# ZINZINBIN/Optimal-Control-1D-Electrostatic-Plasma

Hardware: AMD Instinct MI355X
Metric: particle-steps/sec (N×envs×steps) at N=1e6, Ng=256; % HBM roofline (higher is better)
Workload: dtype f64

## Files before the change

optimal-control-1d-electrostatic-plasma_amd/csrc/pic_device.h:

```cpp
#pragma once
#include <hip/hip_runtime.h>

#include <cmath>
#include <cstdint>
#include <type_traits>

#include "picstep.h"
#include "pic_limits.h"

namespace {

#ifndef PIC_STAMP
#define PIC_STAMP(slot) ((void)0)
#define PIC_STAMP_LOADS(slot) ((void)0)
#endif

constexpr int kInlineDoubles = 32;
struct InlineDoubles { double v[kInlineDoubles]; };

template <typename T>
__device__ __forceinline__ T kernarg_at(size_t offset) {
#if defined(__HIP_DEVICE_COMPILE__)
  using KP = const __attribute__((address_space(4))) char*;
  KP ka = (KP)__builtin_amdgcn_kernarg_segment_ptr();
  asm volatile("" : "+s"(ka));
  T out;
  __builtin_memcpy(&out, (const __attribute__((address_space(4))) T*)(ka + offset), sizeof(T));
  return out;
#else
  (void)offset;
  return T{};
#endif
}

template <typename T>
__device__ __forceinline__ const T* kernarg_ptr(size_t offset) {
#if defined(__HIP_DEVICE_COMPILE__)
  using KP = const __attribute__((address_space(4))) char*;
  KP ka = (KP)__builtin_amdgcn_kernarg_segment_ptr();
  return (const T*)(const char*)(ka + offset);
#else
  (void)offset;
  return nullptr;
#endif
}

template <int BYTES>
__device__ __forceinline__ void kernarg_warm() {
#if defined(__HIP_DEVICE_COMPILE__)
  using KP = const __attribute__((address_space(4))) unsigned*;
  KP ka = (KP)__builtin_amdgcn_kernarg_segment_ptr();
  unsigned w = 0;
#pragma unroll
  for (int line = 1; line < (BYTES + 63) / 64; ++line) w |= ka[line * 16];
  asm volatile("" ::"s"(w));
#endif
}

enum Stage : int {
  ST_A = 0,
  ST_B = 1,
  ST_C = 2,
  ST_D = 3,
  ST_REFRESH = 4,
  ST_PROBE = 5,
  ST_B2 = 6,
  ST_D2 = 7,
  ST_SE = 8,
  ST_FE = 9,
  ST_VK = 10,
  ST_VM = 11,
  ST_C_RO = 12,
  ST_D_RC = 13,
  ST_D2_RC = 14
};

using acc_t = long long;

__device__ __forceinline__ acc_t acc_row_sum(const acc_t* __restrict__ row, int j, int S, long long sub) {
  const acc_t* p = row + j;
  acc_t t = 0;
  int s = 0;
  for (; s + 4 <= S; s += 4) {
    const acc_t r0 = p[0]; p += sub;
    const acc_t r1 = p[0]; p += sub;
    const acc_t r2 = p[0]; p += sub;
    const acc_t r3 = p[0]; p += sub;
    t += (r0 + r1) + (r2 + r3);
  }
  for (; s < S; ++s) { t += p[0]; p += sub; }
  return t;
}

struct SweepArgs {
  long long N;
  long long ld;
  long long chunk;
  int Ng;
  int nblk;
  int R;
  int reverse;
  int fg;
  int S;
  int act_inline;
  long long sub;
  double magic;
  double L, dx, rdx, dt;
  double c_prev, c_cur, d_cur, c_next, d_prev;
  double scale, n0;
  double to_units;
  double N_over_L;
};

struct SolveArgs {
  long long N;
  long long sub;
  int Ng;
  int nblk;
  int fg;
  int S;
  double L, dx, n0;
  double scale;
  double N_over_L;
};

struct AccRequest { acc_t r[4]; };
__device__ __forceinline__ AccRequest acc_row_request(const acc_t* __restrict__ row, int j, int S, long long sub) {
  AccRequest q;
#pragma unroll
  for (int s = 0; s < 4; ++s) q.r[s] = row[(size_t)(s < S ? s : 0) * sub + j];
  return q;
}
__device__ __forceinline__ acc_t acc_row_finish(const AccRequest& q, int S) {
  return (q.r[0] + (S > 1 ? q.r[1] : 0)) + ((S > 2 ? q.r[2] : 0) + (S > 3 ? q.r[3] : 0));
}

struct Control {
  const double* ext;
  const double* act;
  const double* basis;
  int M;
};

__device__ __forceinline__ double actuator_field(const double* __restrict__ bc, const double* __restrict__ bs,
                                                 const double* __restrict__ a, int j, int M) {
  double c = 0.0, s = 0.0;
  for (int m = 0; m < M; ++m) c += bc[(size_t)j * M + m] * a[m];
  for (int m = 0; m < M; ++m) s += bs[(size_t)j * M + m] * a[M + m];
  return c + s;
}

typedef double pic_v2d __attribute__((ext_vector_type(2)));
typedef float pic_v4f __attribute__((ext_vector_type(4)));
typedef unsigned pic_v4u __attribute__((ext_vector_type(4)));

struct PosF64 { using X = double;   using V = double; using W = double; using XV = pic_v2d; using VV = pic_v2d; static constexpr int VEC = 2; static constexpr bool kFixed = false; };
struct PosF32 { using X = float;    using V = float;  using W = float;  using XV = pic_v4f; using VV = pic_v4f; static constexpr int VEC = 4; static constexpr bool kFixed = false; };
struct PosU32 { using X = unsigned; using V = float;  using W = float;  using XV = pic_v4u; using VV = pic_v4f; static constexpr int VEC = 4; static constexpr bool kFixed = true; };

template <typename VT>
__device__ __forceinline__ VT stream_load(const VT* p) { return *p; }

struct StreamOut {
  __amdgpu_buffer_rsrc_t rsrc;
  __device__ explicit StreamOut(void* base) : rsrc(__builtin_amdgcn_make_buffer_rsrc(base, 0, 0x7fffffff, 0x00020000)) {}
  template <typename VT>
  __device__ __forceinline__ void store(int off, VT v) const {
    static_assert(sizeof(VT) == 16, "particle tiles are 16 bytes per lane");
    typedef unsigned pic_v4raw __attribute__((ext_vector_type(4)));
    pic_v4raw w;
    __builtin_memcpy(&w, &v, 16);
    __builtin_amdgcn_raw_buffer_store_b128(w, rsrc, off, 0, 16);
  }
};

template <typename P>
struct Consts {
  typename P::W L, dx, rdx, dt, c_prev, c_cur, d_cur, c_next, d_prev;
  float to_units;
  double magic;
  int Ng;
  __device__ explicit Consts(const SweepArgs& a)
      : L((typename P::W)a.L), dx((typename P::W)a.dx), rdx((typename P::W)a.rdx), dt((typename P::W)a.dt),
        c_prev((typename P::W)a.c_prev), c_cur((typename P::W)a.c_cur), d_cur((typename P::W)a.d_cur),
        c_next((typename P::W)a.c_next), d_prev((typename P::W)a.d_prev), to_units((float)a.to_units), magic(a.magic), Ng(a.Ng) {}
  __device__ Consts(double L_, double dx_, int Ng_)
      : L((typename P::W)L_), dx((typename P::W)dx_), rdx((typename P::W)1 / (typename P::W)dx_), dt(0), c_prev(0),
        c_cur(0), d_cur(0), c_next(0), d_prev(0), to_units((float)(4294967296.0 / L_)), magic(0), Ng(Ng_) {}
};

template <typename T>
__device__ __noinline__ T wrap_periodic_far(T q, T L) {
  T r = fmod(q, L);
  if (r < T(0)) {
    r += L;
    if (r >= L) r = T(0);
  } else if (r == T(0)) {
    r = T(0);
  }
  return r;
}

template <typename T>
__device__ __forceinline__ T wrap_periodic(T q, T L, unsigned& bad) {
  if (__builtin_amdgcn_ballot_w64(!(q > T(0) && q < L)) == 0) return q;
  T up = q + L;
  up = (up >= L) ? T(0) : up;
  T r = (q <= T(0)) ? up : q;
  r = (q >= L) ? q - L : r;
  if (__builtin_expect(!(r >= T(0) && r < L), 0)) {
    r = wrap_periodic_far(q, L);
    if (!(r >= T(0) && r < L)) {
      bad += 1u;
      r = T(0);
    }
  }
  return r;
}

template <typename T>
__device__ __forceinline__ T div_dx(T a, T dx, T rdx) {
  T q0 = a * rdx;
  T rem = fma(-q0, dx, a);
  return fma(rem, rdx, q0);
}

template <typename P, int SHAPE>
__device__ __forceinline__ void locate_in_box(typename P::X xw, const Consts<P>& k, int& j, typename P::W (&w)[3], unsigned& frac) {
  using T = typename P::W;
  static_assert(!P::kFixed, "fixed-point positions need no wrap: locate() is the whole of it");
  frac = 0u;
  T jf = floor(div_dx(xw, k.dx, k.rdx));
  j = (int)jf;
  if ((unsigned)j >= (unsigned)k.Ng) j = 0;
  if (SHAPE == PIC_CIC) {
    w[0] = div_dx((jf + T(1)) * k.dx - xw, k.dx, k.rdx);
    w[1] = div_dx(xw - jf * k.dx, k.dx, k.rdx);
    w[2] = T(0);
  } else {
    T d = div_dx(xw - jf * k.dx, k.dx, k.rdx);
    T a = T(1.5) - d, b = d - T(1), c = d - T(0.5);
    w[0] = T(0.5) * (a * a);
    w[1] = T(0.75) - b * b;
    w[2] = T(0.5) * (c * c);
  }
}

template <typename P, int SHAPE>
__device__ __forceinline__ void locate(typename P::X q, const Consts<P>& k, typename P::X& xw, int& j,
                                       typename P::W (&w)[3], unsigned& frac, unsigned& bad) {
  using T = typename P::W;
  if constexpr (P::kFixed) {
    xw = q;
    j = (int)__umulhi(q, (unsigned)k.Ng);
    frac = q * (unsigned)k.Ng;
    const T d = (T)frac * T(2.3283064365386963e-10);
    if (SHAPE == PIC_CIC) {
      w[1] = d;
      w[0] = T(1) - d;
      w[2] = T(0);
    } else {
      T a = T(1.5) - d, b = d - T(1), c = d - T(0.5);
      w[0] = T(0.5) * (a * a);
      w[1] = T(0.75) - b * b;
      w[2] = T(0.5) * (c * c);
    }
  } else {
    xw = wrap_periodic(q, k.L, bad);
    locate_in_box<P, SHAPE>(xw, k, j, w, frac);
  }
}

template <typename P>
__device__ __forceinline__ double pos_to_length(typename P::X q, double L) {
  if constexpr (P::kFixed) return (double)q * (L * 2.3283064365386963e-10);
  else return (double)q;
}

template <typename P>
__device__ __forceinline__ typename P::X pos_from_length(double xs, double L, unsigned& bad) {
  if constexpr (P::kFixed) {
    double r = xs - floor(xs / L) * L;
    if (!(r >= 0.0 && r < L)) { if (!(r == L)) bad += 1u; r = 0.0; }
    return (unsigned)((unsigned long long)rint(r / L * 4294967296.0) & 0xFFFFFFFFull);
  } else {
    return (typename P::X)xs;
  }
}

template <typename P>
__device__ __forceinline__ typename P::X drift(typename P::X q, typename P::V p, typename P::W c, const Consts<P>& k,
                                               unsigned& bad) {
  using T = typename P::W;
  if constexpr (P::kFixed) {
    const float d = ((c * (T)p) * k.dt) * k.to_units;
    if (!(fabsf(d) < 2147483648.0f)) bad += 1u;
    return q + (unsigned)__float2int_rn(d);
  } else {
    return q + (c * (T)p) * k.dt;
  }
}

template <typename T, int SHAPE>
__device__ __forceinline__ T gather_field(const T* __restrict__ Es, int j, const T (&w)[3]) {
  T e = w[0] * Es[j] + w[1] * Es[j + 1];
  if (SHAPE == PIC_TSC) e = e + w[2] * Es[j + 2];
  return e;
}

struct fix_t { unsigned long long v; };
constexpr int FX_FRAC = 24;
constexpr int FX_LOW = 44;

__device__ __forceinline__ acc_t to_fixed(double w, double magic) {
  return __double_as_longlong(w + magic) - __double_as_longlong(magic);
}

template <typename A, typename P, int SHAPE>
__device__ __forceinline__ void deposit(A* __restrict__ acc, int j, const typename P::W (&w)[3], unsigned frac,
                                        double magic) {
  if constexpr (std::is_same<A, fix_t>::value) {
    static_assert(SHAPE == PIC_CIC, "the packed accumulator is CIC only");
    unsigned long long lo;
    if constexpr (P::kFixed) {
      lo = (frac >> 8) + ((frac >> 7) & 1u);
    } else {
      const float wr = fminf(fmaxf((float)w[1], 0.0f), 1.0f);
      lo = (unsigned long long)(unsigned)(wr * (float)(1u << FX_FRAC) + 0.5f);
    }
    atomicAdd(reinterpret_cast<unsigned long long*>(acc) + j, (1ull << FX_LOW) + lo);
  } else if constexpr (std::is_same<A, acc_t>::value) {
    unsigned long long* a = reinterpret_cast<unsigned long long*>(acc);
    atomicAdd(a + j, (unsigned long long)to_fixed((double)w[0], magic));
    atomicAdd(a + j + 1, (unsigned long long)to_fixed((double)w[1], magic));
    if (SHAPE == PIC_TSC) atomicAdd(a + j + 2, (unsigned long long)to_fixed((double)w[2], magic));
  } else {
    atomicAdd(&acc[j], (A)w[0]);
    atomicAdd(&acc[j + 1], (A)w[1]);
    if (SHAPE == PIC_TSC) atomicAdd(&acc[j + 2], (A)w[2]);
  }
}

template <int CTRL, int ROW_MASK = 0xF>
__device__ __forceinline__ double dpp_add(double v) {
  const int lo = __builtin_amdgcn_update_dpp(0, __double2loint(v), CTRL, ROW_MASK, 0xF, true);
  const int hi = __builtin_amdgcn_update_dpp(0, __double2hiint(v), CTRL, ROW_MASK, 0xF, true);
  return v + __hiloint2double(hi, lo);
}

__device__ __forceinline__ double wave_incl_scan(double v) {
  v = dpp_add<0x111>(v);
  v = dpp_add<0x112>(v);
  v = dpp_add<0x114>(v);
  v = dpp_add<0x118>(v);
  v = dpp_add<0x142, 0xA>(v);
  v = dpp_add<0x143, 0xC>(v);
  return v;
}

__device__ __forceinline__ double wave_sum(double v) {
  v = wave_incl_scan(v);
  const int lo = __builtin_amdgcn_readlane(__double2loint(v), 63);
  const int hi = __builtin_amdgcn_readlane(__double2hiint(v), 63);
  return __hiloint2double(hi, lo);
}

template <int NW>
__device__ __forceinline__ double block_excl_scan(double v, double* ws, double& total) {
  const int lane = threadIdx.x & 63, w = threadIdx.x >> 6;
  double inc = wave_incl_scan(v);
  if (lane == 63) ws[w] = inc;
  __syncthreads();
  double off = 0.0, tot = 0.0;
  for (int i = 0; i < NW; ++i) {
    double s = ws[i];
    if (i < w) off += s;
    tot += s;
  }
  __syncthreads();
  total = tot;
  return off + (inc - v);
}

template <int NW>
__device__ __forceinline__ double block_sum(double v, double* ws) {
  double w = wave_sum(v);
  if ((threadIdx.x & 63) == 0) ws[threadIdx.x >> 6] = w;
  __syncthreads();
  double s = 0.0;
  for (int i = 0; i < NW; ++i) s += ws[i];
  __syncthreads();
  return s;
}

template <int NW>
__device__ __forceinline__ void block_sum2(double a, double b, double* ws, double& sa, double& sb) {
  const double wa = wave_sum(a), wb = wave_sum(b);
  if ((threadIdx.x & 63) == 0) {
    ws[threadIdx.x >> 6] = wa;
    ws[NW + (threadIdx.x >> 6)] = wb;
  }
  __syncthreads();
  sa = 0.0;
  sb = 0.0;
  for (int i = 0; i < NW; ++i) {
    sa += ws[i];
    sb += ws[NW + i];
  }
  __syncthreads();
}

template <int NW>
__device__ __forceinline__ void mesh_mode(const double* __restrict__ E, const double* __restrict__ twc,
                                          const double* __restrict__ tws, int Ng, double* __restrict__ ws, double& re,
                                          double& im) {
  double sr = 0.0, si = 0.0;
  int t0 = threadIdx.x;
  asm volatile("" : "+v"(t0));
  for (int j = t0; j < Ng; j += NW * 64) {
    const double e = E[j];
    sr += e * twc[j];
    si -= e * tws[j];
  }
  double a, b;
  block_sum2<NW>(sr, si, ws, a, b);
  re = a / Ng * 2.0;
  im = b / Ng * 2.0;
}

struct Feedback {
  const double* tw;
  int rows;
  int M;
  double* act_out;
  double* act_hist;
  const double* gain;
  double* modes;
  double* modes_hist;
};

__device__ __forceinline__ double gain_row(const double* __restrict__ g, const double* __restrict__ m, int n) {
  double acc = 0.0;
  bool any = false;
  for (int k = 0; k < n; ++k) {
    const double gk = g[k];
    if (gk != 0.0) {
      const double t = gk * m[k];
      acc = any ? acc + t : t;
      any = true;
    }
  }
  return acc;
}

template <int NW>
__device__ __forceinline__ void feedback_action(const double* __restrict__ E, const Feedback& fb, int env, int Ng,
                                                double* __restrict__ ws, double* __restrict__ a_lds) {
  const size_t r = (size_t)env * 2 * fb.M;
  for (int m = 0; m < fb.M; ++m) {
    double re, im;
    mesh_mode<NW>(E, fb.tw + (size_t)m * Ng, fb.tw + ((size_t)fb.rows + m) * Ng, Ng, ws, re, im);
    if (threadIdx.x == 0) {
      if (fb.gain) {
        double* mv = a_lds ? a_lds : fb.modes + r;
        mv[m] = re; mv[fb.M + m] = im;
        if (fb.modes_hist) { fb.modes_hist[r + m] = re; fb.modes_hist[r + fb.M + m] = im; }
        continue;
      }
      const double c = -re, s = im;
      if (a_lds) { a_lds[m] = c; a_lds[fb.M + m] = s; }
      if (fb.act_out) { fb.act_out[r + m] = c; fb.act_out[r + fb.M + m] = s; }
      if (fb.act_hist) { fb.act_hist[r + m] = c; fb.act_hist[r + fb.M + m] = s; }
    }
  }
  if (fb.gain) {
    __syncthreads();
    const int n = 2 * fb.M;
    int i = threadIdx.x;
    asm volatile("" : "+v"(i));
    const double a = i < n ? gain_row(fb.gain + (r + i) * n, a_lds ? a_lds : fb.modes + r, n) : 0.0;
    if (a_lds) __syncthreads();
    if (i < n) {
      if (a_lds) a_lds[i] = a;
      if (fb.act_out) fb.act_out[r + i] = a;
      if (fb.act_hist) fb.act_hist[r + i] = a;
    }
  }
}

__device__ __forceinline__ void scan_fields(double* __restrict__ sb, double* __restrict__ sp, int Ng, double dx,
                                            double* __restrict__ slot, int wave = 0) {
  if ((int)(threadIdx.x >> 6) != wave) return;
  const int lane = threadIdx.x & 63;
  const int m = (Ng + 63) / 64;
  const int lo = min(lane * m, Ng), hi = min(lo + m, Ng);
  double loc = 0.0;
  for (int j = lo; j < hi; ++j) loc += sb[j];
  double run = wave_incl_scan(loc) - loc;
  loc = 0.0;
  for (int j = lo; j < hi; ++j) {
    run += sb[j];
    const double g = run * dx;
    sb[j] = g;
    loc += g;
  }
  const double gmean = wave_sum(loc) / (double)Ng;
  if (lane == 0) slot[0] = gmean;
  if (sp) {
    loc = 0.0;
    for (int j = lo; j < hi; ++j) loc += (sb[j] - gmean) * dx;
    run = wave_incl_scan(loc) - loc;
    double ploc = 0.0;
    for (int j = lo; j < hi; ++j) {
      sp[j] = run;
      ploc += run;
      run += (sb[j] - gmean) * dx;
    }
    ploc = wave_sum(ploc);
    if (lane == 0) slot[1] = ploc / (double)Ng;
  }
}

struct SolveOut {
  const double* ext;
  double *E, *phi;
  double *KE, *PE, *PEr;
  double* hist;
  int num_envs;
  Feedback fb;
};

template <int NW>
__device__ __forceinline__ void solve_block(const SolveOut& o, int env, int Ng, double dx, double N_over_L, double ke_share,
                                            double* __restrict__ sb, double* __restrict__ se, double* __restrict__ ws,
                                            double* __restrict__ slot) {
  constexpr int NT = NW * 64;
  const int tid = threadIdx.x;
  const size_t row = (size_t)env * Ng;
  scan_fields(sb, o.phi ? se : nullptr, Ng, dx, slot);
  __syncthreads();
  const double gmean = slot[0];
  const double pmean = o.phi ? slot[1] : 0.0;
  double e2 = 0.0;
  for (int j = tid; j < Ng; j += NT) {
    const double gp = sb[j] - gmean;
    const double gm = sb[j == 0 ? Ng - 1 : j - 1] - gmean;
    const double E = -0.5 * (gp + gm);
    const double Et = o.ext ? E + o.ext[row + j] : E;
    if (o.E) o.E[row + j] = Et;
    e2 += Et * Et;
    if (o.phi) o.phi[row + j] = se[j] - pmean;
  }
  double S, K;
  block_sum2<NW>(e2, ke_share, ws, S, K);
  if (tid == 0) {
    const double pe = 0.5 * S * dx;
    if (o.PEr) o.PEr[env] = pe;
    if (o.PE) o.PE[env] = pe * N_over_L;
    if (o.KE) o.KE[env] = 0.5 * K;
    if (o.hist) {
      o.hist[env] = 0.5 * K;
      o.hist[o.num_envs + env] = pe * N_over_L;
      o.hist[2 * (size_t)o.num_envs + env] = pe;
    }
  }
  if (o.fb.M > 0) feedback_action<NW>(o.E + row, o.fb, env, Ng, ws, nullptr);
}

}
```

optimal-control-1d-electrostatic-plasma_amd/csrc/pic_sweep.h:

```cpp
#pragma once
#include "pic_device.h"
#include "pic_solve.h"

namespace {

template <typename T, int OFF>
__device__ __forceinline__ void prologue_field(const acc_t* __restrict__ acc_in, const AccRequest& first, int S, long long sub,
                                               const Control& ctl, double* __restrict__ ext_out, int Ng, double unit, double scale,
                                               double n0, double dx, double* __restrict__ sb, double* __restrict__ xt,
                                               double* __restrict__ slot, T* __restrict__ Es) {
  const int tid = threadIdx.x;
  if (ctl.act)
    for (int j = tid; j < Ng; j += BLOCK) {
      const double e = actuator_field(ctl.basis, ctl.basis + (size_t)Ng * ctl.M, ctl.act, j, ctl.M);
      xt[j] = e;
      if (ext_out) ext_out[j] = e;
    }
  if (tid < Ng) sb[tid] = ((double)acc_row_finish(first, S) * unit) * scale - n0;
  for (int j = tid + BLOCK; j < Ng; j += BLOCK)
    sb[j] = ((double)acc_row_sum(acc_in, j, S, sub) * unit) * scale - n0;
  __syncthreads();
  PIC_STAMP(3);
  scan_fields(sb, nullptr, Ng, dx, slot);
  __syncthreads();
  PIC_STAMP(4);
  const double gmean = slot[0];
  for (int i = tid; i < Ng + 2; i += BLOCK) {
    int node = i - OFF;
    node = node < 0 ? node + Ng : (node >= Ng ? node - Ng : node);
    const double gp = sb[node] - gmean;
    const double gm = sb[node == 0 ? Ng - 1 : node - 1] - gmean;
    double E = -0.5 * (gp + gm);
    if (ctl.act) E += xt[node];
    else if (ctl.ext) E += ctl.ext[node];
    Es[i] = (T)E;
  }
  __syncthreads();
  PIC_STAMP(5);
}

template <typename P, int SHAPE>
__device__ __forceinline__ void substage(typename P::X& q, typename P::V& p, const typename P::W* __restrict__ Es,
                                         typename P::W d, typename P::W c, const Consts<P>& k, unsigned& bad) {
  using T = typename P::W;
  T w[3];
  typename P::X xw;
  int j;
  unsigned frac;
  locate<P, SHAPE>(q, k, xw, j, w, frac, bad);
  const T E = gather_field<T, SHAPE>(Es, j, w);
  p = p + (typename P::V)((d * (-E)) * k.dt);
  q = drift<P>(q, p, c, k, bad);
}

template <typename P, typename A, int SHAPE, int STAGE>
__device__ __forceinline__ void push_one(typename P::X& xq, typename P::V& vp, const typename P::W* __restrict__ Es,
                                         const typename P::W* __restrict__ Es2, A* __restrict__ acc, A* __restrict__ acc2,
                                         const Consts<P>& k, double& ke, unsigned& bad) {
  constexpr bool kC = (STAGE == ST_C || STAGE == ST_C_RO);
  constexpr bool kRC = (STAGE == ST_D_RC || STAGE == ST_D2_RC);
  constexpr bool kD = (STAGE == ST_D || STAGE == ST_D_RC);
  constexpr bool kD2 = (STAGE == ST_D2 || STAGE == ST_D2_RC);
  using T = typename P::W;
  T w[3];
  typename P::X xw;
  int j;
  unsigned frac;
  typename P::X q = xq;
  typename P::V p = vp;
  if (kRC) {
    unsigned again = 0u;
    substage<P, SHAPE>(q, p, Es2, k.d_prev, k.c_prev, k, again);
  }
  if (STAGE == ST_B2) {
    if constexpr (P::kFixed) locate<P, SHAPE>(q, k, xw, j, w, frac, bad);
    else locate_in_box<P, SHAPE>(q, k, j, w, frac);
    deposit<A, P, SHAPE>(acc2, j, w, frac, k.magic);
  }
  if (STAGE == ST_A) {
    q = drift<P>(q, p, k.c_cur, k, bad);
  } else if (STAGE == ST_B || STAGE == ST_B2 || kC || kD || kD2) {
    if (STAGE == ST_B || STAGE == ST_B2) q = drift<P>(q, p, k.c_prev, k, bad);
    substage<P, SHAPE>(q, p, Es, k.d_cur, k.c_cur, k, bad);
  }
  if (kD2) {
    if constexpr (P::kFixed) xw = q;
    else xw = wrap_periodic(q, k.L, bad);
  } else {
    locate<P, SHAPE>(q, k, xw, j, w, frac, bad);
    deposit<A, P, SHAPE>(acc, j, w, frac, k.magic);
  }
  if (kD || kD2 || STAGE == ST_REFRESH) {
    q = xw;
    ke += (double)p * (double)p;
    const typename P::X qn = drift<P>(q, p, k.c_next, k, bad);
    typename P::X xn;
    locate<P, SHAPE>(qn, k, xn, j, w, frac, bad);
    deposit<A, P, SHAPE>(acc2, j, w, frac, k.magic);
  }
  xq = q;
  vp = p;
}

template <typename P, typename A, int SHAPE, int STAGE>
__device__ __forceinline__ void push_scheme(typename P::X& xq, typename P::V& vp, const typename P::W* __restrict__ Es,
                                            A* __restrict__ acc, const Consts<P>& k, double& ke, unsigned& bad) {
  using T = typename P::W;
  using V = typename P::V;
  T w[3];
  typename P::X xw;
  int j;
  unsigned frac;
  typename P::X q = xq;
  V p = vp;
  locate<P, SHAPE>(q, k, xw, j, w, frac, bad);
  const T E = gather_field<T, SHAPE>(Es, j, w);
  if (STAGE == ST_FE) {
    q = drift<P>(xw, p, k.c_cur, k, bad);
    p = p + (V)((k.d_cur * (-E)) * k.dt);
  } else {
    p = p + (V)((k.d_cur * (-E)) * k.dt);
    if (STAGE == ST_VK || STAGE == ST_VM) {
      q = xw;
      ke += (double)p * (double)p;
    }
    if (STAGE == ST_VM) p = p + (V)((k.d_cur * (-E)) * k.dt);
    if (STAGE != ST_VK) q = drift<P>(q, p, k.c_cur, k, bad);
  }
  if (STAGE != ST_VK) {
    locate<P, SHAPE>(q, k, xw, j, w, frac, bad);
    deposit<A, P, SHAPE>(acc, j, w, frac, k.magic);
    if (STAGE != ST_VM) {
      q = xw;
      ke += (double)p * (double)p;
    }
  }
  xq = q;
  vp = p;
}

template <typename A, int SHAPE>
__device__ __forceinline__ acc_t mesh_node_sum(const A* __restrict__ acc_all, int R, int stride, int Ng, int fg, int c) {
  constexpr int OFF = (SHAPE == PIC_TSC) ? 1 : 0;
  if constexpr (std::is_same<A, fix_t>::value) {
    const unsigned long long* a = reinterpret_cast<const unsigned long long*>(acc_all);
    const int cm = c == 0 ? Ng - 1 : c - 1;
    unsigned long long own = 0ull, left = 0ull;
    for (int r = 0; r < R; ++r) {
      own += a[(size_t)r * stride + c];
      left += a[(size_t)r * stride + cm];
    }
    const long long mask = (1ll << FX_LOW) - 1;
    const long long q = ((long long)(own >> FX_LOW) << FX_FRAC) - ((long long)own & mask) + ((long long)left & mask);
    return q << (fg - FX_FRAC);
  } else {
    A s = A(0);
    for (int r = 0; r < R; ++r) {
      const A* ar = acc_all + (size_t)r * stride;
      A t = ar[c + OFF];
      if (SHAPE == PIC_CIC) {
        if (c == 0) t += ar[Ng];
      } else {
        if (c == 0) t += ar[Ng + 1];
        if (c == Ng - 1) t += ar[0];
      }
      s += t;
    }
    if constexpr (std::is_same<A, acc_t>::value) return s;
    else return __double2ll_rn(ldexp((double)s, fg));
  }
}

template <typename A, int SHAPE>
__device__ __forceinline__ void flush_mesh(const A* __restrict__ acc_all, int R, int stride, int Ng, int fg,
                                           acc_t* __restrict__ row) {
  unsigned long long* out = reinterpret_cast<unsigned long long*>(row);
  for (int c = threadIdx.x; c < Ng; c += BLOCK) {
    const acc_t q = mesh_node_sum<A, SHAPE>(acc_all, R, stride, Ng, fg, c);
    if (q) atomicAdd(out + c, (unsigned long long)q);
  }
}

struct SweepIO {
  const acc_t* acc_in;
  Control ctl;
  double* ext_out;
  const double* next_act;
  acc_t* acc_out;
  acc_t* acc_out2;
  acc_t* zero0;
  acc_t* zero1;
  double* ke_part;
  unsigned long long* bad;
  SolveIO post;
  double* e2;
};

constexpr size_t kSweepInlineOffset = 2 * sizeof(void*) + sizeof(SweepIO) + sizeof(SweepArgs);
static_assert(sizeof(SweepIO) % 8 == 0 && sizeof(SweepArgs) % 8 == 0, "arguments lie back to back");

template <typename P, typename A, int SHAPE, int STAGE>
__global__ __launch_bounds__(BLOCK) void sweep_kernel(typename P::X* __restrict__ x, typename P::V* __restrict__ v,
                                                      SweepIO io, SweepArgs a, InlineDoubles act_inline) {
  constexpr int OFF = (SHAPE == PIC_TSC) ? 1 : 0;
  constexpr int VEC = P::VEC;
  using T = typename P::W;
  using XV = typename P::XV;
  using VV = typename P::VV;
  constexpr bool kIsB = (STAGE == ST_B || STAGE == ST_B2), kIsC = (STAGE == ST_C || STAGE == ST_C_RO);
  constexpr bool kRC = (STAGE == ST_D_RC || STAGE == ST_D2_RC);
  constexpr bool kIsD = (STAGE == ST_D || STAGE == ST_D2 || kRC);
  constexpr bool kScheme = (STAGE >= ST_SE && STAGE <= ST_VM);
  constexpr bool kGather = (kIsB || kIsC || kIsD || kScheme);
  constexpr bool kStore = ((kGather && STAGE != ST_C_RO) || STAGE == ST_REFRESH);
  constexpr bool kStoreV = kGather && STAGE != ST_C_RO;
  constexpr bool kAhead = !kStore;
  constexpr bool kReadV = (STAGE != ST_PROBE);
  constexpr bool kFirst = (STAGE != ST_D2 && STAGE != ST_D2_RC && STAGE != ST_VK);
  constexpr bool kDual = (kIsD || STAGE == ST_REFRESH || STAGE == ST_B2);
  constexpr bool kEnergy = (kIsD || STAGE == ST_REFRESH || kScheme);

  extern __shared__ __align__(16) unsigned char smem_raw[];
  const int Ng = a.Ng;
  const int stride = Ng + 2;
  A* acc_all = reinterpret_cast<A*>(smem_raw);
  A* acc2_all = acc_all + (size_t)a.R * stride;
  T* Es = reinterpret_cast<T*>(smem_raw + (size_t)2 * a.R * stride * sizeof(A));
  T* Es2 = Es + stride;
  __shared__ double red[2 * WAVES];
  __shared__ double slot[2];
  static_assert(sizeof(red) + sizeof(slot) == kSweepStaticLds, "pic_create adds the static LDS to the dynamic part it sizes");
  PIC_STAMP(0);

  if (kIsC && blockIdx.x == (unsigned)a.nblk) {
    SolveIO post = kernarg_at<SolveIO>(2 * sizeof(void*) + offsetof(SweepIO, post));
    post.out.fb = Feedback{};
    solve_environment(post, blockIdx.y, Ng, a.nblk, a.fg, a.S, a.sub, a.scale, a.n0, a.dx, a.N_over_L, smem_raw, red, slot);
    return;
  }

  const int tid = threadIdx.x;
  const int env = a.reverse ? (int)gridDim.y - 1 - (int)blockIdx.y : (int)blockIdx.y;
  const int blk = a.reverse ? a.nblk - 1 - (int)blockIdx.x : (int)blockIdx.x;

  typename P::X* xe = x + (size_t)env * a.ld;
  typename P::V* ve = v + (size_t)env * a.ld;
  const long long step = (long long)BLOCK * VEC;
  const long long begin = (long long)blk * a.chunk;
  long long end = begin + a.chunk;
  if (end > a.N) end = a.N;
  long long i = begin + (long long)tid * VEC;
  AccRequest first_node{};
  if (kGather) first_node = acc_row_request(io.acc_in + (size_t)env * Ng, tid < Ng ? tid : Ng - 1, a.S, a.sub);
  const long long i_first = (i + VEC <= end) ? i : 0;
  XV xv = stream_load(reinterpret_cast<const XV*>(xe + i_first));
  VV vv = {};
  if (kReadV) vv = stream_load(reinterpret_cast<const VV*>(ve + i_first));
  PIC_STAMP(2);

  bool clear_first = true;
  if (kGather) {
    Control ctl = io.ctl;
    if (ctl.ext) ctl.ext += (size_t)env * Ng;
    if (a.act_inline) ctl.act = kernarg_ptr<double>(kSweepInlineOffset);
    if (ctl.act) ctl.act += (size_t)env * 2 * ctl.M;
    else {
      for (int c = tid; c < a.R * stride; c += BLOCK) acc_all[c] = A{};
      clear_first = false;
    }
    prologue_field<T, OFF>(io.acc_in + (size_t)env * Ng, first_node, a.S, a.sub, ctl,
                           (io.ext_out && blk == 0) ? io.ext_out + (size_t)env * Ng : nullptr, Ng, ldexp(1.0, -a.fg), a.scale, a.n0, a.dx,
                           reinterpret_cast<double*>(acc2_all), reinterpret_cast<double*>(smem_raw), slot, Es);
  }
  if (STAGE == ST_C_RO && blk == 0)
    for (int c = tid; c < stride; c += BLOCK) io.e2[(size_t)env * stride + c] = (double)Es[c];
  if (kRC)
    for (int c = tid; c < stride; c += BLOCK) Es2[c] = (T)io.e2[(size_t)env * stride + c];
  if (kIsD && io.next_act && io.ext_out && blk == 0) {
    const Control ctl = io.ctl;
    for (int j = tid; j < Ng; j += BLOCK)
      io.ext_out[(size_t)env * Ng + j] = actuator_field(ctl.basis, ctl.basis + (size_t)Ng * ctl.M, io.next_act + (size_t)env * 2 * ctl.M, j, ctl.M);
  }
  if (clear_first) for (int c = tid; c < a.R * stride; c += BLOCK) acc_all[c] = A{};
  if (kDual) for (int c = tid; c < a.R * stride; c += BLOCK) acc2_all[c] = A{};
  if (blk < a.S) {
    const size_t z = (size_t)blk * a.sub + (size_t)env * Ng;
    if (io.zero0) for (int c = tid; c < Ng; c += BLOCK) io.zero0[z + c] = 0;
    if (io.zero1) for (int c = tid; c < Ng; c += BLOCK) io.zero1[z + c] = 0;
  }
  if (clear_first || kDual) __syncthreads();
  PIC_STAMP(6);

  const int rep = (tid >> 6) & (a.R - 1);
  A* acc = acc_all + (size_t)rep * stride;
  A* acc2 = acc2_all + (size_t)rep * stride;
  const Consts<P> k(a);

  double ke = 0.0;
  unsigned bad = 0u;
  [[maybe_unused]] int tile = 0;
  const StreamOut xout(xe + begin), vout(ve + begin);
  while (i + VEC <= end) {
    PIC_STAMP_LOADS(8 + 2 * tile);
    [[maybe_unused]] XV xv_next;
    [[maybe_unused]] VV vv_next = {};
    if constexpr (kAhead) {
      const long long i_next = (i + step + VEC <= end) ? i + step : 0;
      xv_next = stream_load(reinterpret_cast<const XV*>(xe + i_next));
      if (kReadV) vv_next = stream_load(reinterpret_cast<const VV*>(ve + i_next));
    }
    typename P::X* xs = reinterpret_cast<typename P::X*>(&xv);
    typename P::V* vs = reinterpret_cast<typename P::V*>(&vv);
#pragma unroll
    for (int c = 0; c < VEC; ++c) {
      typename P::V pv = kReadV ? vs[c] : typename P::V(0);
      if constexpr (kScheme) push_scheme<P, A, SHAPE, STAGE>(xs[c], pv, Es, acc, k, ke, bad);
      else push_one<P, A, SHAPE, STAGE>(xs[c], pv, Es, Es2, acc, acc2, k, ke, bad);
      if (kReadV) vs[c] = pv;
    }
    if (kStore) {
      xout.store((int)((i - begin) * (long long)sizeof(typename P::X)), xv);
      if (kStoreV) vout.store((int)((i - begin) * (long long)sizeof(typename P::V)), vv);
    }
    PIC_STAMP(9 + 2 * tile);
    ++tile;
    i += step;
    if constexpr (kAhead) {
      xv = xv_next;
      vv = vv_next;
    } else if (i + VEC <= end) {
      xv = stream_load(reinterpret_cast<const XV*>(xe + i));
      if (kReadV) vv = stream_load(reinterpret_cast<const VV*>(ve + i));
    }
  }
  for (long long c = i; c < end; ++c) {
    typename P::X xq = xe[c];
    typename P::V pv = kReadV ? ve[c] : typename P::V(0);
    if constexpr (kScheme) push_scheme<P, A, SHAPE, STAGE>(xq, pv, Es, acc, k, ke, bad);
    else push_one<P, A, SHAPE, STAGE>(xq, pv, Es, Es2, acc, acc2, k, ke, bad);
    if (kStore) {
      xe[c] = xq;
      if (kStoreV) ve[c] = pv;
    }
  }
  __syncthreads();
  PIC_STAMP(24);

  const size_t sub_row = (size_t)(blk % a.S) * a.sub + (size_t)env * Ng;
  if (kFirst) flush_mesh<A, SHAPE>(acc_all, a.R, stride, Ng, a.fg, io.acc_out + sub_row);
  if (kDual) flush_mesh<A, SHAPE>(acc2_all, a.R, stride, Ng, a.fg, io.acc_out2 + sub_row);
  PIC_STAMP(25);

  if (kEnergy) {
    double w = wave_sum(ke);
    if ((tid & 63) == 0) red[tid >> 6] = w;
    __syncthreads();
    if (tid == 0) {
      double s = 0.0;
      for (int c = 0; c < WAVES; ++c) s += red[c];
      io.ke_part[(size_t)env * a.nblk + blk] = s;
    }
  }
  if (bad) atomicAdd(io.bad, (unsigned long long)bad);
  PIC_STAMP_LOADS(26);
}

}
```

Before: 76.51 billion.

## Push particles in lockstep pairs with wave-wide box test and manual double-buffered tiles

For the read-only stages that store nothing, the sweep now double-buffers tile loads explicitly using 32-bit byte offsets. Particles are processed in pairs: one wave-wide compare tests whether every position is strictly inside the box, and only then are locate, gather and deposit interleaved across the pair. Any lane outside the box sends the group back to the full per-particle path. The aim is more instruction-level parallelism and less wrap and branch overhead per particle, at the cost of more register pressure, more code and a possible duplicated fallback path.

```diff
diff --git a/optimal-control-1d-electrostatic-plasma_amd/csrc/pic_device.h b/optimal-control-1d-electrostatic-plasma_amd/csrc/pic_device.h
--- a/optimal-control-1d-electrostatic-plasma_amd/csrc/pic_device.h
+++ b/optimal-control-1d-electrostatic-plasma_amd/csrc/pic_device.h
@@ -218,6 +218,17 @@
   return r;
 }
 
+template <typename T, int N>
+__device__ __forceinline__ bool all_in_open_box(const T (&q)[N], T L) {
+  unsigned long long out = 0ull;
+#pragma unroll
+  for (int c = 0; c < N; ++c) {
+    if constexpr (sizeof(T) == 8) out |= __builtin_amdgcn_fcmp(q[c], T(0), 13) | __builtin_amdgcn_fcmp(q[c], L, 11);
+    else out |= __builtin_amdgcn_fcmpf(q[c], T(0), 13) | __builtin_amdgcn_fcmpf(q[c], L, 11);
+  }
+  return out == 0ull;
+}
+
 template <typename T>
 __device__ __forceinline__ T div_dx(T a, T dx, T rdx) {
   T q0 = a * rdx;
diff --git a/optimal-control-1d-electrostatic-plasma_amd/csrc/pic_sweep.h b/optimal-control-1d-electrostatic-plasma_amd/csrc/pic_sweep.h
--- a/optimal-control-1d-electrostatic-plasma_amd/csrc/pic_sweep.h
+++ b/optimal-control-1d-electrostatic-plasma_amd/csrc/pic_sweep.h
@@ -137,6 +137,141 @@
   }
   xq = q;
   vp = p;
+}
+
+constexpr int kLockstep = 2;
+
+template <typename P, typename A, int SHAPE, int STAGE>
+__device__ __forceinline__ void push_lockstep(const typename P::X* xs, const typename P::V* vs, const typename P::W* __restrict__ Es,
+                                              A* __restrict__ acc, const Consts<P>& k, unsigned& bad) {
+  static_assert(STAGE == ST_A || STAGE == ST_PROBE || STAGE == ST_C_RO, "the stages that store nothing");
+  static_assert(!P::kFixed, "fixed-point positions have no wrap to test");
+  constexpr int G = kLockstep;
+  constexpr bool kReadV = (STAGE != ST_PROBE);
+  using T = typename P::W;
+  using V = typename P::V;
+  typename P::X q[G];
+  V p[G];
+  int j[G];
+  T w[G][3];
+  unsigned frac;
+#pragma unroll
+  for (int c = 0; c < G; ++c) {
+    q[c] = xs[c];
+    p[c] = kReadV ? vs[c] : V(0);
+  }
+  do {
+    if (STAGE == ST_A) {
+#pragma unroll
+      for (int c = 0; c < G; ++c) q[c] = drift<P>(q[c], p[c], k.c_cur, k, bad);
+    } else if (STAGE == ST_C_RO) {
+      if (!all_in_open_box(q, k.L)) break;
+      T E[G];
+#pragma unroll
+      for (int c = 0; c < G; ++c) locate_in_box<P, SHAPE>(q[c], k, j[c], w[c], frac);
+#pragma unroll
+      for (int c = 0; c < G; ++c) E[c] = gather_field<T, SHAPE>(Es, j[c], w[c]);
+#pragma unroll
+      for (int c = 0; c < G; ++c) {
+        p[c] = p[c] + (V)((k.d_cur * (-E[c])) * k.dt);
+        q[c] = drift<P>(q[c], p[c], k.c_cur, k, bad);
+      }
+    }
+    if (!all_in_open_box(q, k.L)) break;
+#pragma unroll
+    for (int c = 0; c < G; ++c) locate_in_box<P, SHAPE>(q[c], k, j[c], w[c], frac);
+#pragma unroll
+    for (int c = 0; c < G; ++c) deposit<A, P, SHAPE>(acc, j[c], w[c], frac, k.magic);
+    return;
+  } while (false);
+  double ke = 0.0;
+#pragma unroll
+  for (int c = 0; c < G; ++c) {
+    typename P::X xq = xs[c];
+    V pv = kReadV ? vs[c] : V(0);
+    asm volatile("" : "+v"(xq), "+v"(pv));
+    push_one<P, A, SHAPE, STAGE>(xq, pv, Es, Es, acc, acc, k, ke, bad);
+  }
+}
+
+template <typename P, typename A, int SHAPE, int STAGE>
+__device__ __forceinline__ void push_tile(const typename P::XV& xv, const typename P::VV& vv, const typename P::W* __restrict__ Es,
+                                          A* __restrict__ acc, const Consts<P>& k, unsigned& bad) {
+  constexpr int VEC = P::VEC;
+  static_assert(VEC % kLockstep == 0, "a tile is whole groups");
+  const typename P::X* xs = reinterpret_cast<const typename P::X*>(&xv);
+  const typename P::V* vs = reinterpret_cast<const typename P::V*>(&vv);
+  if constexpr (P::kFixed) {
+    double ke = 0.0;
+#pragma unroll
+    for (int c = 0; c < VEC; ++c) {
+      typename P::X xq = xs[c];
+      typename P::V pv = (STAGE != ST_PROBE) ? vs[c] : typename P::V(0);
+      push_one<P, A, SHAPE, STAGE>(xq, pv, Es, Es, acc, acc, k, ke, bad);
+    }
+  } else {
+#pragma unroll
+    for (int c = 0; c < VEC; c += kLockstep) push_lockstep<P, A, SHAPE, STAGE>(xs + c, vs + c, Es, acc, k, bad);
+  }
+}
+
+template <typename P, typename A, int SHAPE, int STAGE>
+__device__ __forceinline__ void sweep_tiles_ahead(const typename P::X* __restrict__ xe, const typename P::V* __restrict__ ve,
+                                                  long long begin, long long end, typename P::XV xa, typename P::VV va,
+                                                  const typename P::W* __restrict__ Es, A* __restrict__ acc, const Consts<P>& k,
+                                                  unsigned& bad) {
+  using XV = typename P::XV;
+  using VV = typename P::VV;
+  constexpr int VEC = P::VEC;
+  constexpr bool kReadV = (STAGE != ST_PROBE);
+  constexpr int TILE = BLOCK * VEC;
+  constexpr unsigned kTileBytes = BLOCK * 16u;
+  static_assert(sizeof(typename P::X) == sizeof(typename P::V), "one byte offset serves both arrays");
+  const int tid = threadIdx.x;
+  const long long len = end > begin ? end - begin : 0;
+  const int nfull = (int)(len / TILE);
+  const int rem = (int)(len - (long long)nfull * TILE);
+  const bool part = tid * VEC + VEC <= rem;
+  const long long base = len > 0 ? begin : 0;
+  const char* xb = reinterpret_cast<const char*>(xe + base);
+  const char* vb = reinterpret_cast<const char*>(ve + base);
+  const unsigned lane = (unsigned)tid * 16u;
+  const unsigned off_part = part ? lane + (unsigned)nfull * kTileBytes : 0u;
+  auto request = [&](unsigned off, XV& xr, VV& vr) {
+    xr = stream_load(reinterpret_cast<const XV*>(xb + off));
+    if (kReadV) vr = stream_load(reinterpret_cast<const VV*>(vb + off));
+  };
+  XV xn;
+  VV vn = {};
+  int t = 0;
+  for (; t + 2 <= nfull; t += 2) {
+    PIC_STAMP_LOADS(8 + 2 * t);
+    request(lane + (unsigned)(t + 1) * kTileBytes, xn, vn);
+    push_tile<P, A, SHAPE, STAGE>(xa, va, Es, acc, k, bad);
+    PIC_STAMP(9 + 2 * t);
+    PIC_STAMP_LOADS(10 + 2 * t);
+    request(t + 2 < nfull ? lane + (unsigned)(t + 2) * kTileBytes : off_part, xa, va);
+    push_tile<P, A, SHAPE, STAGE>(xn, vn, Es, acc, k, bad);
+    PIC_STAMP(11 + 2 * t);
+  }
+  if (t < nfull) {
+    PIC_STAMP_LOADS(8 + 2 * t);
+    request(off_part, xn, vn);
+    push_tile<P, A, SHAPE, STAGE>(xa, va, Es, acc, k, bad);
+    PIC_STAMP(9 + 2 * t);
+    xa = xn;
+    va = vn;
+  }
+  if (part) {
+    push_tile<P, A, SHAPE, STAGE>(xa, va, Es, acc, k, bad);
+  } else {
+    for (long long c = begin + (long long)nfull * TILE + (long long)tid * VEC; c < end; ++c) {
+      typename P::X xq = xe[c];
+      typename P::V pv = kReadV ? ve[c] : typename P::V(0);
+      double ke = 0.0;
+      push_one<P, A, SHAPE, STAGE>(xq, pv, Es, Es, acc, acc, k, ke, bad);
+    }
+  }
 }
 
 template <typename A, int SHAPE>
@@ -298,47 +433,37 @@
 
   double ke = 0.0;
   unsigned bad = 0u;
-  [[maybe_unused]] int tile = 0;
-  const StreamOut xout(xe + begin), vout(ve + begin);
-  while (i + VEC <= end) {
-    PIC_STAMP_LOADS(8 + 2 * tile);
-    [[maybe_unused]] XV xv_next;
-    [[maybe_unused]] VV vv_next = {};
-    if constexpr (kAhead) {
-      const long long i_next = (i + step + VEC <= end) ? i + step : 0;
-      xv_next = stream_load(reinterpret_cast<const XV*>(xe + i_next));
-      if (kReadV) vv_next = stream_load(reinterpret_cast<const VV*>(ve + i_next));
-    }
-    typename P::X* xs = reinterpret_cast<typename P::X*>(&xv);
-    typename P::V* vs = reinterpret_cast<typename P::V*>(&vv);
-#pragma unroll
-    for (int c = 0; c < VEC; ++c) {
-      typename P::V pv = kReadV ? vs[c] : typename P::V(0);
-      if constexpr (kScheme) push_scheme<P, A, SHAPE, STAGE>(xs[c], pv, Es, acc, k, ke, bad);
-      else push_one<P, A, SHAPE, STAGE>(xs[c], pv, Es, Es2, acc, acc2, k, ke, bad);
-      if (kReadV) vs[c] = pv;
-    }
-    if (kStore) {
+  if constexpr (kAhead) {
+    sweep_tiles_ahead<P, A, SHAPE, STAGE>(xe, ve, begin, end, xv, vv, Es, acc, k, bad);
+  } else {
+    int tile = 0;
+    const StreamOut xout(xe + begin), vout(ve + begin);
+    while (i + VEC <= end) {
+      PIC_STAMP_LOADS(8 + 2 * tile);
+      typename P::X* xs = reinterpret_cast<typename P::X*>(&xv);
+      typename P::V* vs = reinterpret_cast<typename P::V*>(&vv);
+#pragma unroll
+      for (int c = 0; c < VEC; ++c) {
+        typename P::V pv = kReadV ? vs[c] : typename P::V(0);
+        if constexpr (kScheme) push_scheme<P, A, SHAPE, STAGE>(xs[c], pv, Es, acc, k, ke, bad);
+        else push_one<P, A, SHAPE, STAGE>(xs[c], pv, Es, Es2, acc, acc2, k, ke, bad);
+        if (kReadV) vs[c] = pv;
+      }
       xout.store((int)((i - begin) * (long long)sizeof(typename P::X)), xv);
       if (kStoreV) vout.store((int)((i - begin) * (long long)sizeof(typename P::V)), vv);
-    }
-    PIC_STAMP(9 + 2 * tile);
-    ++tile;
-    i += step;
-    if constexpr (kAhead) {
-      xv = xv_next;
-      vv = vv_next;
-    } else if (i + VEC <= end) {
-      xv = stream_load(reinterpret_cast<const XV*>(xe + i));
-      if (kReadV) vv = stream_load(reinterpret_cast<const VV*>(ve + i));
-    }
-  }
-  for (long long c = i; c < end; ++c) {
-    typename P::X xq = xe[c];
-    typename P::V pv = kReadV ? ve[c] : typename P::V(0);
-    if constexpr (kScheme) push_scheme<P, A, SHAPE, STAGE>(xq, pv, Es, acc, k, ke, bad);
-    else push_one<P, A, SHAPE, STAGE>(xq, pv, Es, Es2, acc, acc2, k, ke, bad);
-    if (kStore) {
+      PIC_STAMP(9 + 2 * tile);
+      ++tile;
+      i += step;
+      if (i + VEC <= end) {
+        xv = stream_load(reinterpret_cast<const XV*>(xe + i));
+        if (kReadV) vv = stream_load(reinterpret_cast<const VV*>(ve + i));
+      }
+    }
+    for (long long c = i; c < end; ++c) {
+      typename P::X xq = xe[c];
+      typename P::V pv = kReadV ? ve[c] : typename P::V(0);
+      if constexpr (kScheme) push_scheme<P, A, SHAPE, STAGE>(xq, pv, Es, acc, k, ke, bad);
+      else push_one<P, A, SHAPE, STAGE>(xq, pv, Es, Es2, acc, acc2, k, ke, bad);
       xe[c] = xq;
       if (kStoreV) ve[c] = pv;
     }
```

After: 70.41 billion. 8.0% lower.
